# TUMFTM/DPFT

Hardware: AMD Instinct MI355X
Metric: training samples/sec (K-Radar C+R, bs4/GPU) (higher is better)
Workload: dtype f32

## Files before the change

### dpft_amd/csrc/decoder_train_x.hip

```cpp
#include "common.h"
#include "decoder_pack.h"
#include <stdlib.h>

namespace dpft {

constexpr int XR_DLIN = 0;
constexpr int XR_DF = XR_DLIN + NOA;
constexpr int XR_DPRE = XR_DF + 16;
constexpr int XR_DOUT = XR_DPRE + 32;
constexpr int XR_G3 = XR_DOUT + 16;
constexpr int XR_B3 = XR_G3 + 16;
constexpr int XR_G2 = XR_B3 + 16;
constexpr int XR_B2 = XR_G2 + 16;
constexpr int XR_DBV = XR_B2 + 16;
constexpr int XR_DVEC = XR_DBV + 16;
constexpr int XR_SUMMED = XR_DVEC + 16;
constexpr int XR_QP = XR_SUMMED;
constexpr int XR_HD = XR_QP + 16;
constexpr int XR_Y2 = XR_HD + 32;
constexpr int XR_VEC = XR_Y2 + 16;
constexpr int XR_SAMP = XR_VEC + 16;
constexpr int XR_FLOATS = XR_SAMP + 128;

struct Pyr5g {
    const float* level[DPFT_MAX_LEVELS];
    float* grad[DPFT_MAX_LEVELS];
    int H[DPFT_MAX_LEVELS], W[DPFT_MAX_LEVELS];
    int rep[DPFT_MAX_LEVELS];
    int L;
};
struct XfArgs {
    Pyr5g pyr[4];
    const float* pv[4];
    dpft_decoder_view raw[4];
    const float* y1;
    const float* pos;
    const float* ref;
    const int64_t* seed;
    float* y3;
    const float* dy3;
    float* dy1;
    float* dqp;
    float* dref;
    float* rows;
    float* fsave;
    float* scratch;
    signed char slot[4][DPFT_MAX_LEVELS];
    int B, Q, salt;
    int P[4];
    float p_drop;
    int exp;
};
constexpr int XS_ACC = 0;
constexpr int XS_MS = 128;
constexpr int XS_FLOATS = 136;
constexpr int XC_DS = 0;
constexpr int XC_SLOT = 128;
constexpr int XC_SLOT_FLOATS = 160;
constexpr int XC_MAX_SLOTS = 5;
constexpr int XC_FLOATS = XC_SLOT + XC_MAX_SLOTS * XC_SLOT_FLOATS;
constexpr int XC_MAX_PIXELS = 2048;

__device__ __forceinline__ uint32_t xdrop_hash(uint32_t idx, uint32_t s0, uint32_t s1) {
    uint32_t x = idx ^ s0;
    x *= 0xcc9e2d51u; x = (x << 15) | (x >> 17); x *= 0x1b873593u;
    x ^= s1;
    x ^= x >> 16; x *= 0x85ebca6bu; x ^= x >> 13; x *= 0xc2b2ae35u; x ^= x >> 16;
    return x;
}
__device__ __forceinline__ float xdrop_scale(const int64_t* seed, int salt, int stream_id, float p, uint32_t e) {
    const uint64_t s = (uint64_t)(*seed);
    const uint32_t s0 = (uint32_t)s ^ ((uint32_t)salt * 0x9E3779B9u);
    const uint32_t s1 = (uint32_t)(s >> 32) + (uint32_t)stream_id * 0x7F4A7C15u;
    const uint32_t thr = (uint32_t)(p * 65536.f + 0.5f);
    const uint32_t h = xdrop_hash(e >> 1, s0, s1);
    return ((h >> (16 * (e & 1))) & 0xFFFFu) >= thr ? 1.f / (1.f - p) : 0.f;
}

template <int CTRL>
__device__ __forceinline__ float xdpp(float v) {
    return __builtin_bit_cast(float, __builtin_amdgcn_update_dpp(0, __builtin_bit_cast(int, v), CTRL, 0xF, 0xF, false));
}
__device__ __forceinline__ float xg8_sum(float v) {
    v += xdpp<0xB1>(v);
    v += xdpp<0x4E>(v);
    v += xdpp<0x141>(v);
    return v;
}
__device__ __forceinline__ float xg16_sum(float v) {
    v = xg8_sum(v);
    v += xdpp<0x140>(v);
    return v;
}

struct XfFwd {
    float y1c;
    float mx, inv_den;
    float rx, ry;
    f32x2 acc;
    float ms;
    float vecc;
    float k2, y2, zhat2, rstd2;
    float pre, k3, hd;
    float k4, zhat3, rstd3, y3;
};

template <bool SAVED>
__device__ __forceinline__ void xf_forward_row(const XfArgs& a, int view, int bq, int b, int q, int lane, float* qp,
                                               float* lin, float* vec, XfFwd& f) {
    const float* pv = a.pv[view];
    const Pyr5g& pyr = a.pyr[view];
    const int L = pyr.L, P = a.P[view], LP = L * P;
    const size_t vbq = (size_t)view * a.B * a.Q + bq;
    const int c = lane & 15;
    f.y1c = a.y1[vbq * DC + c];
    if (lane < 16) qp[lane] = f.y1c + a.pos[(size_t)q * DC + lane];
    __builtin_amdgcn_wave_barrier();
    const int n_off = DM * LP * 2, n_all = DM * LP * 3;
    {
        float x[DC];
#pragma unroll
        for (int k = 0; k < DC; ++k) x[k] = qp[k];
        for (int o = lane; o < n_all; o += 64) {
            float s = pv[PV_OA_B + o];
#pragma unroll
            for (int k = 0; k < DC; ++k) s = fmaf(pv[PV_OA_WT + k * NOA + o], x[k], s);
            lin[o] = s;
        }
    }
    __builtin_amdgcn_wave_barrier();
    const int m = lane >> 3, j = lane & 7;
    const float* lg = lin + n_off + m * LP;
    float mx = -INFINITY;
    for (int i = 0; i < LP; ++i) mx = fmaxf(mx, lg[i]);
    float den = 0.f;
    for (int i = 0; i < LP; ++i) den += __expf(lg[i] - mx);
    f.mx = mx;
    f.inv_den = 1.f / den;
    f.rx = a.ref[vbq * 2 + 0];
    f.ry = a.ref[vbq * 2 + 1];
    const float* offp = lin + m * LP * 2;
    f32x2 acc = {0.f, 0.f};
    float ms = 0.f;
    if (SAVED) {
        const float* sv = a.fsave + vbq * XS_FLOATS;
        acc = *reinterpret_cast<const f32x2*>(sv + XS_ACC + m * DC + j * 2);
        ms = sv[XS_MS + m];
    }
    for (int l = 0; !SAVED && l < L; ++l) {
        const int H = pyr.H[l], W = pyr.W[l];
        const float* base = pyr.level[l] + (int64_t)b * H * W * DC + j * 2;
        f32x2 v[4][4];
        float wgt[4][4];
#pragma unroll
        for (int p = 0; p < 4; ++p) {
            const bool act = p < P;
            const int lp = act ? l * P + p : l * P;
            const float ox = offp[lp * 2 + 0], oy = offp[lp * 2 + 1];
            const float aw = act ? __expf(lg[lp] - mx) * f.inv_den : 0.f;
            const float lx = f.rx + ox / (float)W, ly = f.ry + oy / (float)H;
            const float h_im = ly * H - 0.5f, w_im = lx * W - 0.5f;
            const bool in = act && h_im > -1 && w_im > -1 && h_im < H && w_im < W;
            const float hf = floorf(h_im), wf = floorf(w_im);
            const int h_lo = (int)hf, w_lo = (int)wf, h_hi = h_lo + 1, w_hi = w_lo + 1;
            const float lh = h_im - hf, lw = w_im - wf, hh = 1 - lh, hw = 1 - lw;
            const bool k1 = in && h_lo >= 0 && w_lo >= 0, k2 = in && h_lo >= 0 && w_hi <= W - 1;
            const bool k3 = in && h_hi <= H - 1 && w_lo >= 0, k4 = in && h_hi <= H - 1 && w_hi <= W - 1;
            const int hl = min(max(h_lo, 0), H - 1), hh_ = min(max(h_hi, 0), H - 1);
            const int wl = min(max(w_lo, 0), W - 1), wh_ = min(max(w_hi, 0), W - 1);
            v[p][0] = *reinterpret_cast<const f32x2*>(base + ((int64_t)hl * W + wl) * DC);
            v[p][1] = *reinterpret_cast<const f32x2*>(base + ((int64_t)hl * W + wh_) * DC);
            v[p][2] = *reinterpret_cast<const f32x2*>(base + ((int64_t)hh_ * W + wl) * DC);
            v[p][3] = *reinterpret_cast<const f32x2*>(base + ((int64_t)hh_ * W + wh_) * DC);
            wgt[p][0] = k1 ? aw * hh * hw : 0.f;
            wgt[p][1] = k2 ? aw * hh * lw : 0.f;
            wgt[p][2] = k3 ? aw * lh * hw : 0.f;
            wgt[p][3] = k4 ? aw * lh * lw : 0.f;
        }
#pragma unroll
        for (int p = 0; p < 4; ++p)
#pragma unroll
            for (int k = 0; k < 4; ++k) {
                acc += wgt[p][k] * v[p][k];
                ms += wgt[p][k];
            }
    }
    f.acc = acc;
    f.ms = ms;
    const f32x2 wv0 = *reinterpret_cast<const f32x2*>(pv + PV_VAL_W + (m * DD + 0) * DC + j * 2);
    const f32x2 wv1 = *reinterpret_cast<const f32x2*>(pv + PV_VAL_W + (m * DD + 1) * DC + j * 2);
    const float o0 = xg8_sum(wv0[0] * acc[0] + wv0[1] * acc[1]);
    const float o1 = xg8_sum(wv1[0] * acc[0] + wv1[1] * acc[1]);
    if (j == 0) {
        vec[m * 2 + 0] = o0 + pv[PV_VAL_B + m * 2 + 0] * ms;
        vec[m * 2 + 1] = o1 + pv[PV_VAL_B + m * 2 + 1] * ms;
    }
    __builtin_amdgcn_wave_barrier();
    f.vecc = vec[c];
    float vo = pv[PV_OUTP_B + c];
#pragma unroll
    for (int k = 0; k < DC; ++k) vo = fmaf(pv[PV_OUTP_WT + k * DC + c], vec[k], vo);
    f.k2 = xdrop_scale(a.seed, a.salt, 2, a.p_drop, (uint32_t)(vbq * DC + c));
    vo = f.y1c + vo * f.k2;
    {
        const float mean = xg16_sum(vo) * (1.f / 16.f);
        const float d = vo - mean;
        const float var = xg16_sum(d * d) * (1.f / 16.f);
        f.rstd2 = 1.0f / sqrtf(var + 1e-5f);
        f.zhat2 = d * f.rstd2;
        f.y2 = f.zhat2 * pv[PV_N2_W + c] + pv[PV_N2_B + c];
    }
    __builtin_amdgcn_wave_barrier();
    if (lane < 16) qp[lane] = f.y2;
    __builtin_amdgcn_wave_barrier();
    {
        const int jf = lane & 31;
        float hsum = pv[PV_F1_B + jf];
#pragma unroll
        for (int k = 0; k < DC; ++k) hsum = fmaf(pv[PV_F1_WT + k * DFF + jf], qp[k], hsum);
        f.pre = hsum;
        f.k3 = xdrop_scale(a.seed, a.salt, 3, a.p_drop, (uint32_t)(vbq * DFF + jf));
        f.hd = mishf(hsum) * f.k3;
        if (lane < DFF) vec[lane] = f.hd;
    }
    __builtin_amdgcn_wave_barrier();
    float ff = pv[PV_F2_B + c];
#pragma unroll
    for (int k = 0; k < DFF; ++k) ff = fmaf(pv[PV_F2_WT + k * DC + c], vec[k], ff);
    f.k4 = xdrop_scale(a.seed, a.salt, 4, a.p_drop, (uint32_t)(vbq * DC + c));
    ff = f.y2 + ff * f.k4;
    {
        const float mean = xg16_sum(ff) * (1.f / 16.f);
        const float d = ff - mean;
        const float var = xg16_sum(d * d) * (1.f / 16.f);
        f.rstd3 = 1.0f / sqrtf(var + 1e-5f);
        f.zhat3 = d * f.rstd3;
        f.y3 = f.zhat3 * pv[PV_N3_W + c] + pv[PV_N3_B + c];
    }
}

constexpr int XF_WAVES = 5;
__global__ __launch_bounds__(256) void xf_train_fwd_kernel(XfArgs a) {
    __shared__ float sm[4][16 + NOA + 32];
    const int lane = threadIdx.x & 63, wv = __builtin_amdgcn_readfirstlane(threadIdx.x >> 6);
    const int bq = blockIdx.x * 4 + wv, view = blockIdx.y;
    if (bq >= a.B * a.Q) return;
    const int b = bq / a.Q, q = bq - b * a.Q;
    float* qp = sm[wv];
    XfFwd f;
    xf_forward_row<false>(a, view, bq, b, q, lane, qp, qp + 16, qp + 16 + NOA, f);
    const size_t vbq = (size_t)view * a.B * a.Q + bq;
    if (lane < 16) a.y3[vbq * DC + lane] = f.y3;
    if (a.fsave) {
        float* sv = a.fsave + vbq * XS_FLOATS;
        *reinterpret_cast<f32x2*>(sv + XS_ACC + (lane >> 3) * DC + (lane & 7) * 2) = f.acc;
        if ((lane & 7) == 0) sv[XS_MS + (lane >> 3)] = f.ms;
    }
}

template <bool SAVED>
__global__ __launch_bounds__(256, XF_WAVES) void xf_train_bwd_kernel(XfArgs a) {
    __shared__ __attribute__((aligned(16))) float sm[4][16 + NOA + 32 + NOA + 32 + 32 + 128 + 128 + 32];
    const int lane = threadIdx.x & 63, wv = __builtin_amdgcn_readfirstlane(threadIdx.x >> 6);
    const int bq = blockIdx.x * 4 + wv, view = blockIdx.y;
    if (bq >= a.B * a.Q) return;
    const int b = bq / a.Q, q = bq - b * a.Q;
    float* qp = sm[wv];
    float* lin = qp + 16;
    float* vec = lin + NOA;
    float* dlin = vec + 32;
    float* va = dlin + NOA;
    float* vb2 = va + 32;
    float* ds16 = vb2 + 32;
    float* sc_w = ds16 + 128;
    int* sc_o = reinterpret_cast<int*>(sc_w + 128);
    XfFwd f;
    xf_forward_row<SAVED>(a, view, bq, b, q, lane, qp, lin, vec, f);
    const float* pv = a.pv[view];
    const dpft_decoder_view& rw = a.raw[view];
    const Pyr5g& pyr = a.pyr[view];
    const int L = pyr.L, P = a.P[view], LP = L * P;
    const int n_off = DM * LP * 2, n_all = DM * LP * 3;
    const size_t vbq = (size_t)view * a.B * a.Q + bq;
    float* row = a.rows + vbq * XR_FLOATS;
    const int c = lane & 15, m = lane >> 3, j = lane & 7, jf = lane & 31;
    const bool w16 = lane < 16, w32 = lane < 32;
    const float dy3 = a.dy3[vbq * DC + c];
    float dzh = dy3 * pv[PV_N3_W + c];
    float m1 = xg16_sum(dzh) * (1.f / 16.f), m2 = xg16_sum(dzh * f.zhat3) * (1.f / 16.f);
    const float dz3 = f.rstd3 * (dzh - m1 - f.zhat3 * m2);
    const float df = dz3 * f.k4;
    if (w16) {
        row[XR_G3 + c] = dy3 * f.zhat3;
        row[XR_B3 + c] = dy3;
        row[XR_DF + c] = df;
        row[XR_Y2 + c] = f.y2;
        va[c] = df;
    }
    if (w32) row[XR_HD + jf] = f.hd;
    __builtin_amdgcn_wave_barrier();
    float dhd = 0.f;
#pragma unroll 4
    for (int k = 0; k < DC; ++k) dhd = fmaf(va[k], rw.ffn2_w[k * DFF + jf], dhd);
    float dpre;
    {
        const float x = f.pre;
        const float sp = x > 20.f ? x : log1pf(expf(x));
        const float t = tanhf(sp);
        const float sg = 1.f / (1.f + expf(-x));
        dpre = dhd * f.k3 * (t + x * (1.f - t * t) * sg);
    }
    if (w32) {
        row[XR_DPRE + jf] = dpre;
        vb2[jf] = dpre;
    }
    __builtin_amdgcn_wave_barrier();
    float dy2 = dz3;
#pragma unroll 4
    for (int k = 0; k < DFF; ++k) dy2 = fmaf(vb2[k], rw.ffn1_w[k * DC + c], dy2);
    dzh = dy2 * pv[PV_N2_W + c];
    m1 = xg16_sum(dzh) * (1.f / 16.f);
    m2 = xg16_sum(dzh * f.zhat2) * (1.f / 16.f);
    const float dz2 = f.rstd2 * (dzh - m1 - f.zhat2 * m2);
    const float dout = dz2 * f.k2;
    __builtin_amdgcn_wave_barrier();
    if (w16) {
        row[XR_G2 + c] = dy2 * f.zhat2;
        row[XR_B2 + c] = dy2;
        row[XR_DOUT + c] = dout;
        row[XR_VEC + c] = f.vecc;
        va[c] = dout;
    }
    __builtin_amdgcn_wave_barrier();
    float dvec = 0.f;
#pragma unroll 4
    for (int k = 0; k < DC; ++k) dvec = fmaf(va[k], rw.outp_w[k * DC + c], dvec);
    {
        const float msk = __shfl(f.ms, (c >> 1) * 8);
        if (w16) {
            row[XR_DVEC + c] = dvec;
            row[XR_DBV + c] = dvec * msk;
            vb2[c] = dvec;
        }
    }
    *reinterpret_cast<f32x2*>(row + XR_SAMP + m * DC + j * 2) = f.acc;
    __builtin_amdgcn_wave_barrier();
    const float g0 = vb2[m * DD + 0], g1 = vb2[m * DD + 1];
    const f32x2 w0 = *reinterpret_cast<const f32x2*>(pv + PV_VAL_W + (m * DD + 0) * DC + j * 2);
    const f32x2 w1v = *reinterpret_cast<const f32x2*>(pv + PV_VAL_W + (m * DD + 1) * DC + j * 2);
    const f32x2 dS = {w0[0] * g0 + w1v[0] * g1, w0[1] * g0 + w1v[1] * g1};
    const float dM = pv[PV_VAL_B + m * DD + 0] * g0 + pv[PV_VAL_B + m * DD + 1] * g1;
    *reinterpret_cast<f32x2*>(ds16 + m * DC + j * 2) = dS;
    float* rec = a.scratch ? a.scratch + vbq * XC_FLOATS : nullptr;
    if (rec) *reinterpret_cast<f32x2*>(rec + XC_DS + m * DC + j * 2) = dS;
    const float* lg = lin + n_off + m * LP;
    const float* offp = lin + m * LP * 2;
    float* dlg = dlin + n_off + m * LP;
    float* doff = dlin + m * LP * 2;
    float grx = 0.f, gry = 0.f, sdot = 0.f;
    for (int l = 0; l < L; ++l) {
        const int H = pyr.H[l], W = pyr.W[l];
        const float* base = pyr.level[l] + (int64_t)b * H * W * DC + j * 2;
        f32x2 v[4][4];
        float aw[4], hh[4], hw[4], lh[4], lw[4];
        bool kk[4][4];
#pragma unroll
        for (int p = 0; p < 4; ++p) {
            const bool act = p < P;
            const int lp = act ? l * P + p : l * P;
            const float ox = offp[lp * 2 + 0], oy = offp[lp * 2 + 1];
            aw[p] = act ? __expf(lg[lp] - f.mx) * f.inv_den : 0.f;
            const float lx = f.rx + ox / (float)W, ly = f.ry + oy / (float)H;
            const float h_im = ly * H - 0.5f, w_im = lx * W - 0.5f;
            const bool in = act && h_im > -1 && w_im > -1 && h_im < H && w_im < W;
            const float hf = floorf(h_im), wf = floorf(w_im);
            const int h_lo = (int)hf, w_lo = (int)wf, h_hi = h_lo + 1, w_hi = w_lo + 1;
            lh[p] = h_im - hf; lw[p] = w_im - wf; hh[p] = 1 - lh[p]; hw[p] = 1 - lw[p];
            kk[p][0] = in && h_lo >= 0 && w_lo >= 0;     kk[p][1] = in && h_lo >= 0 && w_hi <= W - 1;
            kk[p][2] = in && h_hi <= H - 1 && w_lo >= 0; kk[p][3] = in && h_hi <= H - 1 && w_hi <= W - 1;
            const int hl = min(max(h_lo, 0), H - 1), hh_ = min(max(h_hi, 0), H - 1);
            const int wl = min(max(w_lo, 0), W - 1), wh_ = min(max(w_hi, 0), W - 1);
            v[p][0] = *reinterpret_cast<const f32x2*>(base + ((int64_t)hl * W + wl) * DC);
            v[p][1] = *reinterpret_cast<const f32x2*>(base + ((int64_t)hl * W + wh_) * DC);
            v[p][2] = *reinterpret_cast<const f32x2*>(base + ((int64_t)hh_ * W + wl) * DC);
            v[p][3] = *reinterpret_cast<const f32x2*>(base + ((int64_t)hh_ * W + wh_) * DC);
            if (j == 0) {
                const float w1 = hh[p] * hw[p], w2 = hh[p] * lw[p], w3 = lh[p] * hw[p], w4 = lh[p] * lw[p];
                *reinterpret_cast<f32x4*>(sc_w + (p * 8 + m) * 4) =
                    f32x4{kk[p][0] ? aw[p] * w1 : 0.f, kk[p][1] ? aw[p] * w2 : 0.f, kk[p][2] ? aw[p] * w3 : 0.f,
                          kk[p][3] ? aw[p] * w4 : 0.f};
                sc_o[p * 8 + m] = in ? (h_lo * W + w_lo) * DC : 0;
            }
        }
#pragma unroll
        for (int p = 0; p < 4; ++p) {
            if (p >= P) break;
            const int lp = l * P + p;
            const float w1 = hh[p] * hw[p], w2 = hh[p] * lw[p], w3 = lh[p] * hw[p], w4 = lh[p] * lw[p];
            float ga = 0.f, gw = 0.f, gh = 0.f;
#pragma unroll
            for (int e = 0; e < 2; ++e) {
                const float v1 = kk[p][0] ? v[p][0][e] : 0.f, v2 = kk[p][1] ? v[p][1][e] : 0.f;
                const float v3 = kk[p][2] ? v[p][2][e] : 0.f, v4 = kk[p][3] ? v[p][3][e] : 0.f;
                ga += dS[e] * (w1 * v1 + w2 * v2 + w3 * v3 + w4 * v4);
                gh += dS[e] * aw[p] * (-hw[p] * v1 - lw[p] * v2 + hw[p] * v3 + lw[p] * v4);
                gw += dS[e] * aw[p] * (-hh[p] * v1 + hh[p] * v2 - lh[p] * v3 + lh[p] * v4);
            }
            if (j == 0) {
                const float i1 = kk[p][0] ? 1.f : 0.f, i2 = kk[p][1] ? 1.f : 0.f, i3 = kk[p][2] ? 1.f : 0.f, i4 = kk[p][3] ? 1.f : 0.f;
                ga += dM * (w1 * i1 + w2 * i2 + w3 * i3 + w4 * i4);
                gh += dM * aw[p] * (-hw[p] * i1 - lw[p] * i2 + hw[p] * i3 + lw[p] * i4);
                gw += dM * aw[p] * (-hh[p] * i1 + hh[p] * i2 - lh[p] * i3 + lh[p] * i4);
            }
            ga = xg8_sum(ga);
            gw = xg8_sum(gw);
            gh = xg8_sum(gh);
            sdot = fmaf(aw[p], ga, sdot);
            if (j == 0) {
                dlg[lp] = ga;
                doff[lp * 2 + 0] = gw;
                doff[lp * 2 + 1] = gh;
                grx = fmaf((float)W, gw, grx);
                gry = fmaf((float)H, gh, gry);
            }
        }
        __builtin_amdgcn_wave_barrier();
        const int slot = rec ? (int)a.slot[view][l] : -1;
        if (slot >= 0) {
            float* dst = rec + XC_SLOT + slot * XC_SLOT_FLOATS;
            if (lane < 32) reinterpret_cast<f32x4*>(dst)[lane] = reinterpret_cast<const f32x4*>(sc_w)[lane];
            else reinterpret_cast<int*>(dst + 128)[lane - 32] = sc_o[lane - 32];
        } else if (!(a.exp & 1)) {
            float* gl = pyr.grad[l] + (int64_t)(bq % pyr.rep[l]) * a.B * H * W * DC + (int64_t)b * H * W * DC;
            const int h4 = lane >> 4, ch = lane & 15, W16 = W * DC;
#pragma unroll
            for (int half = 0; half < 2; ++half) {
                const int m2 = h4 + 4 * half;
                const float val = ds16[m2 * DC + ch];
#pragma unroll
                for (int p = 0; p < 4; ++p) {
                    const f32x4 cw = *reinterpret_cast<const f32x4*>(sc_w + (p * 8 + m2) * 4);
                    float* g00 = gl + sc_o[p * 8 + m2] + ch;
                    if (cw[0] != 0.f) atomicAdd(g00, cw[0] * val);
                    if (cw[1] != 0.f) atomicAdd(g00 + DC, cw[1] * val);
                    if (cw[2] != 0.f) atomicAdd(g00 + W16, cw[2] * val);
                    if (cw[3] != 0.f) atomicAdd(g00 + W16 + DC, cw[3] * val);
                }
            }
        }
        __builtin_amdgcn_wave_barrier();
    }
    __builtin_amdgcn_wave_barrier();
    for (int lp = j; lp < LP; lp += 8) {
        const float awp = __expf(lg[lp] - f.mx) * f.inv_den;
        dlg[lp] = awp * (dlg[lp] - sdot);
    }
    {
        float sx = grx, sy = gry;
#pragma unroll
        for (int o = 8; o < 64; o <<= 1) {
            sx += __shfl_xor(sx, o);
            sy += __shfl_xor(sy, o);
        }
        if (lane == 0) {
            a.dref[vbq * 2 + 0] = sx;
            a.dref[vbq * 2 + 1] = sy;
        }
    }
    __builtin_amdgcn_wave_barrier();
    for (int o = lane; o < NOA; o += 64) row[XR_DLIN + o] = o < n_all ? dlin[o] : 0.f;
    const float qpc = f.y1c + a.pos[(size_t)q * DC + c];
    if (w16) row[XR_QP + c] = qpc;
    float dq = 0.f;
    {
        const int part = lane >> 4;
        for (int o = part; o < n_all; o += 4) {
            const float wgt = o < n_off ? rw.off_w[o * DC + c] : rw.att_w[(o - n_off) * DC + c];
            dq = fmaf(dlin[o], wgt, dq);
        }
        dq += __shfl_xor(dq, 16);
        dq += __shfl_xor(dq, 32);
    }
    if (w16) {
        a.dqp[vbq * DC + c] = dq;
        a.dy1[vbq * DC + c] = dz2 + dq;
    }
}

struct XsArgs {
    const float* scratch;
    float* grad[4 * XC_MAX_SLOTS];
    int H[4 * XC_MAX_SLOTS], W[4 * XC_MAX_SLOTS], view[4 * XC_MAX_SLOTS], slot[4 * XC_MAX_SLOTS];
    int B, Q, qchunk;
    int exp;
};
__global__ __launch_bounds__(512) void xf_scatter_small_kernel(XsArgs a) {
    extern __shared__ __attribute__((aligned(16))) float img[];
    const int tid = threadIdx.x, lane = tid & 63, wave = __builtin_amdgcn_readfirstlane(tid >> 6);
    const int mi = blockIdx.y, b = blockIdx.z;
    const int H = a.H[mi], W = a.W[mi], view = a.view[mi], slot = a.slot[mi];
    const int n = H * W * DC, W16 = W * DC;
    for (int i = tid * 4; i < n; i += 512 * 4) *reinterpret_cast<f32x4*>(img + i) = f32x4{0.f, 0.f, 0.f, 0.f};
    __syncthreads();
    const int q0 = blockIdx.x * a.qchunk, q1 = min(a.Q, q0 + a.qchunk);
    const int h4 = lane >> 4, ch = lane & 15;
    for (int q = q0 + wave; q < q1 && !(a.exp & 8); q += 8) {
        const float* rec = a.scratch + (((size_t)view * a.B + b) * a.Q + q) * XC_FLOATS;
        const float* wrec = rec + XC_SLOT + slot * XC_SLOT_FLOATS;
        const int* orec = reinterpret_cast<const int*>(wrec + 128);
        float val[2];
        f32x4 cw[2][4];
        int off[2][4];
#pragma unroll
        for (int half = 0; half < 2; ++half) {
            const int m2 = h4 + 4 * half;
            val[half] = rec[XC_DS + m2 * DC + ch];
#pragma unroll
            for (int p = 0; p < 4; ++p) {
                cw[half][p] = *reinterpret_cast<const f32x4*>(wrec + (p * 8 + m2) * 4);
                off[half][p] = orec[p * 8 + m2];
            }
        }
        if (a.exp & 2) {
            float acc = val[0] + val[1];
            for (int half = 0; half < 2; ++half)
                for (int p = 0; p < 4; ++p) acc += cw[half][p][0] + cw[half][p][3] + (float)off[half][p];
            if (acc == 12345.678f) img[0] = acc;
            continue;
        }
#pragma unroll
        for (int half = 0; half < 2; ++half)
#pragma unroll
            for (int p = 0; p < 4; ++p) {
                float* g00 = img + off[half][p] + ch;
                const f32x4 w4 = cw[half][p];
                if (w4[0] != 0.f) atomicAdd(g00, w4[0] * val[half]);
                if (w4[1] != 0.f) atomicAdd(g00 + DC, w4[1] * val[half]);
                if (w4[2] != 0.f) atomicAdd(g00 + W16, w4[2] * val[half]);
                if (w4[3] != 0.f) atomicAdd(g00 + W16 + DC, w4[3] * val[half]);
            }
    }
    __syncthreads();
    float* g = a.grad[mi] + (size_t)b * n;
    for (int i = tid; i < n && !(a.exp & 4); i += 512) {
        const float v = img[i];
        if (v != 0.f) atomicAdd(g + i, v);
    }
}

}

using namespace dpft;

static int xf_fill(XfArgs& a, const dpft_pyramid* pyr, const dpft_decoder_view* views, const float* packed, int V,
                   const int32_t* n_points, const float* y1, const float* pos, const float* ref, float p_drop,
                   const int64_t* seed, int salt, int B, int Q, bool need_grad) {
    DPFT_REQUIRE(pyr && views && packed && n_points && y1 && pos && ref && seed, "xattn_ffn_train: null argument");
    DPFT_REQUIRE(V >= 1 && V <= 4 && B > 0 && Q > 0, "xattn_ffn_train: bad sizes (V=%d, B=%d, Q=%d)", V, B, Q);
    DPFT_REQUIRE(p_drop >= 0.f && p_drop < 1.f, "xattn_ffn_train: dropout probability must be in [0,1)");
    DPFT_REQUIRE((int64_t)V * B * Q * DFF < (1ll << 32), "xattn_ffn_train: problem too large for the mask index");
    memset(&a, 0, sizeof(a));
    memset(a.slot, -1, sizeof(a.slot));
    for (int v = 0; v < V; ++v) {
        const dpft_pyramid* p = pyr + v;
        const int P = n_points[v];
        DPFT_REQUIRE(p->L >= 1 && p->L <= DPFT_MAX_LEVELS && P >= 1 && P <= 4 && p->L * P * DM * 3 <= NOA,
                     "xattn_ffn_train: L=%d, P=%d exceed the fused kernel's budget (P <= 4, L*P <= 20)", p->L, P);
        a.pyr[v].L = p->L;
        for (int l = 0; l < p->L; ++l) {
            DPFT_REQUIRE(p->level[l] && p->H[l] > 0 && p->W[l] > 0, "xattn_ffn_train: view %d level %d is invalid", v, l);
            DPFT_REQUIRE(!need_grad || p->grad[l], "xattn_ffn_train: view %d level %d has no gradient buffer", v, l);
            DPFT_REQUIRE((int64_t)p->H[l] * p->W[l] * DC < (1ll << 31), "xattn_ffn_train: view %d level %d is too large", v, l);
            a.pyr[v].level[l] = p->level[l]; a.pyr[v].grad[l] = p->grad[l];
            a.pyr[v].rep[l] = p->grad_replicas[l] > 1 ? p->grad_replicas[l] : 1;
            a.pyr[v].H[l] = p->H[l]; a.pyr[v].W[l] = p->W[l];
        }
        a.P[v] = P;
        a.pv[v] = packed + (size_t)v * PV_FLOATS;
        a.raw[v] = views[v];
    }
    a.y1 = y1; a.pos = pos; a.ref = ref; a.seed = seed; a.salt = salt; a.p_drop = p_drop; a.B = B; a.Q = Q;
    return DPFT_OK;
}

extern "C" int64_t dpft_xattn_ffn_train_row_floats(void) { return XR_FLOATS; }
extern "C" int64_t dpft_xattn_ffn_train_saved_floats(void) { return XS_FLOATS; }
extern "C" int64_t dpft_xattn_ffn_train_scratch_floats(void) { return XC_FLOATS; }

extern "C" int dpft_xattn_ffn_train_fwd_f32(const dpft_pyramid* pyr, const dpft_decoder_view* views, const float* packed,
                                            int32_t V, const int32_t* n_points, const float* y1, const float* pos,
                                            const float* ref, float p_drop, const int64_t* seed, int32_t salt, float* y3,
                                            float* saved, int32_t B, int32_t Q, dpft_stream_t stream) {
    XfArgs a;
    int rc = xf_fill(a, pyr, views, packed, V, n_points, y1, pos, ref, p_drop, seed, salt, B, Q, false);
    if (rc) return rc;
    DPFT_REQUIRE(y3, "xattn_ffn_train_fwd: null output");
    a.y3 = y3;
    a.fsave = saved;
    hipLaunchKernelGGL(xf_train_fwd_kernel, dim3(cdiv((int64_t)B * Q, 4), V), dim3(256), 0, (hipStream_t)stream, a);
    return check_launch("xattn_ffn_train_fwd");
}

extern "C" int dpft_xattn_ffn_train_bwd_f32(const dpft_pyramid* pyr, const dpft_decoder_view* views, const float* packed,
                                            int32_t V, const int32_t* n_points, const float* y1, const float* pos,
                                            const float* ref, float p_drop, const int64_t* seed, int32_t salt,
                                            const float* saved, const float* dy3, float* dy1, float* dqp, float* dref,
                                            float* rows, float* scratch, int32_t B, int32_t Q, dpft_stream_t stream) {
    XfArgs a;
    int rc = xf_fill(a, pyr, views, packed, V, n_points, y1, pos, ref, p_drop, seed, salt, B, Q, true);
    if (rc) return rc;
    DPFT_REQUIRE(dy3 && dy1 && dqp && dref && rows, "xattn_ffn_train_bwd: null argument");
    a.dy3 = dy3; a.dy1 = dy1; a.dqp = dqp; a.dref = dref; a.rows = rows;
    a.fsave = const_cast<float*>(saved);
    static const int exp = getenv("DPFT_XF_EXP") ? atoi(getenv("DPFT_XF_EXP")) : 0;
    a.exp = exp;
    XsArgs xs;
    memset(&xs, 0, sizeof(xs));
    int n_maps = 0, max_px = 0;
    static const bool allow = !(getenv("DPFT_XF_SCATTER") && atoi(getenv("DPFT_XF_SCATTER")) == 0);
    if (scratch && allow) {
        a.scratch = scratch;
        for (int v = 0; v < V; ++v) {
            int order[DPFT_MAX_LEVELS], n = 0;
            for (int l = 0; l < a.pyr[v].L; ++l)
                if (a.pyr[v].H[l] * a.pyr[v].W[l] <= XC_MAX_PIXELS && a.pyr[v].rep[l] == 1) order[n++] = l;
            for (int i = 1; i < n; ++i)
                for (int k = i; k > 0 && a.pyr[v].H[order[k]] * a.pyr[v].W[order[k]] < a.pyr[v].H[order[k - 1]] * a.pyr[v].W[order[k - 1]]; --k) {
                    const int t = order[k]; order[k] = order[k - 1]; order[k - 1] = t;
                }
            for (int i = 0; i < n && i < XC_MAX_SLOTS; ++i) {
                const int l = order[i];
                a.slot[v][l] = (signed char)i;
                xs.grad[n_maps] = a.pyr[v].grad[l];
                xs.H[n_maps] = a.pyr[v].H[l]; xs.W[n_maps] = a.pyr[v].W[l];
                xs.view[n_maps] = v; xs.slot[n_maps] = i;
                max_px = max_px > xs.H[n_maps] * xs.W[n_maps] ? max_px : xs.H[n_maps] * xs.W[n_maps];
                ++n_maps;
            }
        }
        if (n_maps == 0) a.scratch = nullptr;
    }
    if (saved)
        hipLaunchKernelGGL(xf_train_bwd_kernel<true>, dim3(cdiv((int64_t)B * Q, 4), V), dim3(256), 0, (hipStream_t)stream, a);
    else
        hipLaunchKernelGGL(xf_train_bwd_kernel<false>, dim3(cdiv((int64_t)B * Q, 4), V), dim3(256), 0, (hipStream_t)stream, a);
    rc = check_launch("xattn_ffn_train_bwd");
    if (rc || n_maps == 0) return rc;
    int nchunk = kNumCU / (n_maps * B);
    nchunk = nchunk < 1 ? 1 : (nchunk > 8 ? 8 : nchunk);
    xs.scratch = scratch; xs.B = B; xs.Q = Q; xs.qchunk = cdiv(Q, nchunk); xs.exp = exp;
    nchunk = cdiv(Q, xs.qchunk);
    const size_t lds = (size_t)max_px * DC * sizeof(float);
    static LdsGrant grant;
    (void)lds_grant(grant, reinterpret_cast<const void*>(xf_scatter_small_kernel), (size_t)XC_MAX_PIXELS * DC * sizeof(float));
    hipLaunchKernelGGL(xf_scatter_small_kernel, dim3(nchunk, n_maps, B), dim3(512), lds, (hipStream_t)stream, xs);
    return check_launch("xattn_ffn_train_bwd (small-map scatter)");
}
```

Baseline: 171.0.

## Stage decoder weights in LDS, vectorize GEMVs, and prefetch scatter records

Each block of the cross-attention forward and backward kernels now stages the value, out-projection, FFN and norm parameters into padded shared memory, and every per-row GEMV reads from there instead of global memory. The offset/attention linear layer is vectorized to float4 with register pinning. The dq reduction is split into chunked dot products, and the scatter path uses LDS address-space pointers plus an int-word read of the slot table. The small-scatter kernel software-pipelines record loads by prefetching the next query. These changes aim to cut global-memory and latency costs, at the price of a block-wide sync, extra LDS use and more register pressure.

Measured after the change: 167.0. 2.4% lower.

```diff
diff --git a/dpft_amd/csrc/decoder_train_x.hip b/dpft_amd/csrc/decoder_train_x.hip
--- a/dpft_amd/csrc/decoder_train_x.hip
+++ b/dpft_amd/csrc/decoder_train_x.hip
@@ -1,5 +1,6 @@
 #include "common.h"
 #include "decoder_pack.h"
+#include <stddef.h>
 #include <stdlib.h>
 
 namespace dpft {
@@ -68,8 +69,7 @@
     x ^= x >> 16; x *= 0x85ebca6bu; x ^= x >> 13; x *= 0xc2b2ae35u; x ^= x >> 16;
     return x;
 }
-__device__ __forceinline__ float xdrop_scale(const int64_t* seed, int salt, int stream_id, float p, uint32_t e) {
-    const uint64_t s = (uint64_t)(*seed);
+__device__ __forceinline__ float xdrop_scale(uint64_t s, int salt, int stream_id, float p, uint32_t e) {
     const uint32_t s0 = (uint32_t)s ^ ((uint32_t)salt * 0x9E3779B9u);
     const uint32_t s1 = (uint32_t)(s >> 32) + (uint32_t)stream_id * 0x7F4A7C15u;
     const uint32_t thr = (uint32_t)(p * 65536.f + 0.5f);
@@ -105,31 +105,107 @@
     float k4, zhat3, rstd3, y3;
 };
 
+constexpr int SW_VAL = 0;
+constexpr int SW_OUTP = SW_VAL + 272;
+constexpr int SW_F1 = SW_OUTP + 16 * 17;
+constexpr int SW_F2 = SW_F1 + 16 * 33;
+constexpr int SW_OUTP_B = SW_F2 + 32 * 17;
+constexpr int SW_N2_W = SW_OUTP_B + 16;
+constexpr int SW_N2_B = SW_N2_W + 16;
+constexpr int SW_F1_B = SW_N2_B + 16;
+constexpr int SW_F2_B = SW_F1_B + 32;
+constexpr int SW_N3_W = SW_F2_B + 16;
+constexpr int SW_N3_B = SW_N3_W + 16;
+constexpr int SW_FLOATS = SW_N3_B + 16;
+static_assert(PV_VAL_B == PV_VAL_W + 256 && PV_OUTP_WT == PV_VAL_W + 272 && PV_OUTP_B == PV_OUTP_WT + 256 &&
+              PV_F1_WT == PV_OUTP_B + 48 && PV_F1_B == PV_F1_WT + 512 && PV_F2_WT == PV_F1_B + 32 &&
+              PV_F2_B == PV_F2_WT + 512 && PV_FLOATS == PV_F2_B + 48 && PV_VAL_W % 4 == 0 && PV_FLOATS % 4 == 0 &&
+              PV_OA_WT % 4 == 0 && NOA % 4 == 0, "xf_stage_params / the float4 GEMV follow the packed layout");
+
+__device__ __forceinline__ int xf_stage_index(int r) {
+    constexpr int R_OUTP = PV_OUTP_WT - PV_VAL_W, R_OUTP_B = PV_OUTP_B - PV_VAL_W, R_F1 = PV_F1_WT - PV_VAL_W;
+    constexpr int R_F1_B = PV_F1_B - PV_VAL_W, R_F2 = PV_F2_WT - PV_VAL_W, R_F2_B = PV_F2_B - PV_VAL_W;
+    if (r < R_OUTP) return SW_VAL + r;
+    if (r < R_OUTP_B) return SW_OUTP + ((r - R_OUTP) >> 4) * 17 + ((r - R_OUTP) & 15);
+    if (r < R_F1) return SW_OUTP_B + (r - R_OUTP_B);
+    if (r < R_F1_B) return SW_F1 + ((r - R_F1) >> 5) * 33 + ((r - R_F1) & 31);
+    if (r < R_F2) return SW_F1_B + (r - R_F1_B);
+    if (r < R_F2_B) return SW_F2 + ((r - R_F2) >> 4) * 17 + ((r - R_F2) & 15);
+    return SW_F2_B + (r - R_F2_B);
+}
+__device__ __forceinline__ void xf_stage_params(const float* pv, float* sw) {
+    constexpr int N4 = (PV_FLOATS - PV_VAL_W) / 4;
+    const f32x4* src = reinterpret_cast<const f32x4*>(pv + PV_VAL_W);
+    const int t = threadIdx.x;
+    const f32x4 v0 = src[t];
+    const f32x4 v1 = src[t + 256 < N4 ? t + 256 : t];
+    const int d0 = xf_stage_index(t * 4);
+#pragma unroll
+    for (int e = 0; e < 4; ++e) sw[d0 + e] = v0[e];
+    if (t + 256 < N4) {
+        const int d1 = xf_stage_index((t + 256) * 4);
+#pragma unroll
+        for (int e = 0; e < 4; ++e) sw[d1 + e] = v1[e];
+    }
+    __syncthreads();
+}
+static_assert((PV_FLOATS - PV_VAL_W) / 4 > 256 && (PV_FLOATS - PV_VAL_W) / 4 <= 512, "xf_stage_params: two loads per thread");
+
+__device__ __forceinline__ void xf_pin8(f32x4 (&w)[8]) {
+    asm volatile("" : "+v"(w[0]), "+v"(w[1]), "+v"(w[2]), "+v"(w[3]), "+v"(w[4]), "+v"(w[5]), "+v"(w[6]), "+v"(w[7]));
+}
+typedef __attribute__((address_space(3))) const float xf_lds_f;
+typedef __attribute__((address_space(3))) const int xf_lds_i;
+template <class T>
+__device__ __forceinline__ T* xf_lds_pin(const void* p) {
+    T* q = (T*)p;
+    asm volatile("" : "+v"(q));
+    return q;
+}
+
 template <bool SAVED>
 __device__ __forceinline__ void xf_forward_row(const XfArgs& a, int view, int bq, int b, int q, int lane, float* qp,
-                                               float* lin, float* vec, XfFwd& f) {
+                                               float* lin, float* vec, const float* sw, XfFwd& f) {
     const float* pv = a.pv[view];
     const Pyr5g& pyr = a.pyr[view];
     const int L = pyr.L, P = a.P[view], LP = L * P;
     const size_t vbq = (size_t)view * a.B * a.Q + bq;
     const int c = lane & 15;
+    const int m = lane >> 3, j = lane & 7;
     f.y1c = a.y1[vbq * DC + c];
-    if (lane < 16) qp[lane] = f.y1c + a.pos[(size_t)q * DC + lane];
+    const float posc = a.pos[(size_t)q * DC + c];
+    f.rx = a.ref[vbq * 2 + 0];
+    f.ry = a.ref[vbq * 2 + 1];
+    const uint64_t seed = (uint64_t)(*a.seed);
+    f32x2 acc = {0.f, 0.f};
+    float ms = 0.f;
+    if (SAVED) {
+        const float* sv = a.fsave + vbq * XS_FLOATS;
+        acc = *reinterpret_cast<const f32x2*>(sv + XS_ACC + m * DC + j * 2);
+        ms = sv[XS_MS + m];
+    }
+    if (lane < 16) qp[lane] = f.y1c + posc;
     __builtin_amdgcn_wave_barrier();
     const int n_off = DM * LP * 2, n_all = DM * LP * 3;
-    {
-        float x[DC];
-#pragma unroll
-        for (int k = 0; k < DC; ++k) x[k] = qp[k];
-        for (int o = lane; o < n_all; o += 64) {
-            float s = pv[PV_OA_B + o];
-#pragma unroll
-            for (int k = 0; k < DC; ++k) s = fmaf(pv[PV_OA_WT + k * NOA + o], x[k], s);
-            lin[o] = s;
-        }
-    }
-    __builtin_amdgcn_wave_barrier();
-    const int m = lane >> 3, j = lane & 7;
+    for (int o = lane * 4; o < n_all; o += 256) {
+        const float* wt = pv + PV_OA_WT + o;
+        f32x4 s = *reinterpret_cast<const f32x4*>(pv + PV_OA_B + o);
+#pragma unroll
+        for (int k0 = 0; k0 < DC; k0 += 8) {
+            f32x4 w[8];
+#pragma unroll
+            for (int k = 0; k < 8; ++k) w[k] = *reinterpret_cast<const f32x4*>(wt + (k0 + k) * NOA);
+            xf_pin8(w);
+#pragma unroll
+            for (int k = 0; k < 8; ++k) {
+                const float x = qp[k0 + k];
+#pragma unroll
+                for (int e = 0; e < 4; ++e) s[e] = fmaf(w[k][e], x, s[e]);
+            }
+        }
+        *reinterpret_cast<f32x4*>(lin + o) = s;
+    }
+    __builtin_amdgcn_wave_barrier();
     const float* lg = lin + n_off + m * LP;
     float mx = -INFINITY;
     for (int i = 0; i < LP; ++i) mx = fmaxf(mx, lg[i]);
@@ -137,16 +213,7 @@
     for (int i = 0; i < LP; ++i) den += __expf(lg[i] - mx);
     f.mx = mx;
     f.inv_den = 1.f / den;
-    f.rx = a.ref[vbq * 2 + 0];
-    f.ry = a.ref[vbq * 2 + 1];
     const float* offp = lin + m * LP * 2;
-    f32x2 acc = {0.f, 0.f};
-    float ms = 0.f;
-    if (SAVED) {
-        const float* sv = a.fsave + vbq * XS_FLOATS;
-        acc = *reinterpret_cast<const f32x2*>(sv + XS_ACC + m * DC + j * 2);
-        ms = sv[XS_MS + m];
-    }
     for (int l = 0; !SAVED && l < L; ++l) {
         const int H = pyr.H[l], W = pyr.W[l];
         const float* base = pyr.level[l] + (int64_t)b * H * W * DC + j * 2;
@@ -187,20 +254,20 @@
     }
     f.acc = acc;
     f.ms = ms;
-    const f32x2 wv0 = *reinterpret_cast<const f32x2*>(pv + PV_VAL_W + (m * DD + 0) * DC + j * 2);
-    const f32x2 wv1 = *reinterpret_cast<const f32x2*>(pv + PV_VAL_W + (m * DD + 1) * DC + j * 2);
+    const f32x2 wv0 = *reinterpret_cast<const f32x2*>(sw + SW_VAL + (m * DD + 0) * DC + j * 2);
+    const f32x2 wv1 = *reinterpret_cast<const f32x2*>(sw + SW_VAL + (m * DD + 1) * DC + j * 2);
     const float o0 = xg8_sum(wv0[0] * acc[0] + wv0[1] * acc[1]);
     const float o1 = xg8_sum(wv1[0] * acc[0] + wv1[1] * acc[1]);
     if (j == 0) {
-        vec[m * 2 + 0] = o0 + pv[PV_VAL_B + m * 2 + 0] * ms;
-        vec[m * 2 + 1] = o1 + pv[PV_VAL_B + m * 2 + 1] * ms;
+        vec[m * 2 + 0] = o0 + sw[SW_VAL + 256 + m * 2 + 0] * ms;
+        vec[m * 2 + 1] = o1 + sw[SW_VAL + 256 + m * 2 + 1] * ms;
     }
     __builtin_amdgcn_wave_barrier();
     f.vecc = vec[c];
-    float vo = pv[PV_OUTP_B + c];
-#pragma unroll
-    for (int k = 0; k < DC; ++k) vo = fmaf(pv[PV_OUTP_WT + k * DC + c], vec[k], vo);
-    f.k2 = xdrop_scale(a.seed, a.salt, 2, a.p_drop, (uint32_t)(vbq * DC + c));
+    float vo = sw[SW_OUTP_B + c];
+#pragma unroll
+    for (int k = 0; k < DC; ++k) vo = fmaf(sw[SW_OUTP + k * 17 + c], vec[k], vo);
+    f.k2 = xdrop_scale(seed, a.salt, 2, a.p_drop, (uint32_t)(vbq * DC + c));
     vo = f.y1c + vo * f.k2;
     {
         const float mean = xg16_sum(vo) * (1.f / 16.f);
@@ -208,26 +275,26 @@
         const float var = xg16_sum(d * d) * (1.f / 16.f);
         f.rstd2 = 1.0f / sqrtf(var + 1e-5f);
         f.zhat2 = d * f.rstd2;
-        f.y2 = f.zhat2 * pv[PV_N2_W + c] + pv[PV_N2_B + c];
+        f.y2 = f.zhat2 * sw[SW_N2_W + c] + sw[SW_N2_B + c];
     }
     __builtin_amdgcn_wave_barrier();
     if (lane < 16) qp[lane] = f.y2;
     __builtin_amdgcn_wave_barrier();
     {
         const int jf = lane & 31;
-        float hsum = pv[PV_F1_B + jf];
-#pragma unroll
-        for (int k = 0; k < DC; ++k) hsum = fmaf(pv[PV_F1_WT + k * DFF + jf], qp[k], hsum);
+        float hsum = sw[SW_F1_B + jf];
+#pragma unroll
+        for (int k = 0; k < DC; ++k) hsum = fmaf(sw[SW_F1 + k * 33 + jf], qp[k], hsum);
         f.pre = hsum;
-        f.k3 = xdrop_scale(a.seed, a.salt, 3, a.p_drop, (uint32_t)(vbq * DFF + jf));
+        f.k3 = xdrop_scale(seed, a.salt, 3, a.p_drop, (uint32_t)(vbq * DFF + jf));
         f.hd = mishf(hsum) * f.k3;
         if (lane < DFF) vec[lane] = f.hd;
     }
     __builtin_amdgcn_wave_barrier();
-    float ff = pv[PV_F2_B + c];
-#pragma unroll
-    for (int k = 0; k < DFF; ++k) ff = fmaf(pv[PV_F2_WT + k * DC + c], vec[k], ff);
-    f.k4 = xdrop_scale(a.seed, a.salt, 4, a.p_drop, (uint32_t)(vbq * DC + c));
+    float ff = sw[SW_F2_B + c];
+#pragma unroll
+    for (int k = 0; k < DFF; ++k) ff = fmaf(sw[SW_F2 + k * 17 + c], vec[k], ff);
+    f.k4 = xdrop_scale(seed, a.salt, 4, a.p_drop, (uint32_t)(vbq * DC + c));
     ff = f.y2 + ff * f.k4;
     {
         const float mean = xg16_sum(ff) * (1.f / 16.f);
@@ -235,20 +302,22 @@
         const float var = xg16_sum(d * d) * (1.f / 16.f);
         f.rstd3 = 1.0f / sqrtf(var + 1e-5f);
         f.zhat3 = d * f.rstd3;
-        f.y3 = f.zhat3 * pv[PV_N3_W + c] + pv[PV_N3_B + c];
+        f.y3 = f.zhat3 * sw[SW_N3_W + c] + sw[SW_N3_B + c];
     }
 }
 
 constexpr int XF_WAVES = 5;
 __global__ __launch_bounds__(256) void xf_train_fwd_kernel(XfArgs a) {
-    __shared__ float sm[4][16 + NOA + 32];
+    __shared__ __attribute__((aligned(16))) float sm[4][16 + NOA + 32];
+    __shared__ float sw[SW_FLOATS];
     const int lane = threadIdx.x & 63, wv = __builtin_amdgcn_readfirstlane(threadIdx.x >> 6);
     const int bq = blockIdx.x * 4 + wv, view = blockIdx.y;
+    xf_stage_params(a.pv[view], sw);
     if (bq >= a.B * a.Q) return;
     const int b = bq / a.Q, q = bq - b * a.Q;
     float* qp = sm[wv];
     XfFwd f;
-    xf_forward_row<false>(a, view, bq, b, q, lane, qp, qp + 16, qp + 16 + NOA, f);
+    xf_forward_row<false>(a, view, bq, b, q, lane, qp, qp + 16, qp + 16 + NOA, sw, f);
     const size_t vbq = (size_t)view * a.B * a.Q + bq;
     if (lane < 16) a.y3[vbq * DC + lane] = f.y3;
     if (a.fsave) {
@@ -258,11 +327,30 @@
     }
 }
 
+template <int CH>
+__device__ __forceinline__ float xf_dot_chunk(const float* w, const float* d, float dq) {
+    float t[CH];
+#pragma unroll
+    for (int u = 0; u < CH; ++u) t[u] = w[u * 4 * DC];
+#pragma unroll
+    for (int u = 0; u < CH; ++u) dq = fmaf(d[u * 4], t[u], dq);
+    return dq;
+}
+__device__ __forceinline__ float xf_dot_rows(const float* w, const float* d, int n, float dq) {
+    int i = 0;
+    for (; i + 16 <= n; i += 16) dq = xf_dot_chunk<16>(w + i * 4 * DC, d + i * 4, dq);
+    for (; i + 4 <= n; i += 4) dq = xf_dot_chunk<4>(w + i * 4 * DC, d + i * 4, dq);
+    for (; i < n; i += 2) dq = xf_dot_chunk<2>(w + i * 4 * DC, d + i * 4, dq);
+    return dq;
+}
+
 template <bool SAVED>
 __global__ __launch_bounds__(256, XF_WAVES) void xf_train_bwd_kernel(XfArgs a) {
     __shared__ __attribute__((aligned(16))) float sm[4][16 + NOA + 32 + NOA + 32 + 32 + 128 + 128 + 32];
+    __shared__ float sw[SW_FLOATS];
     const int lane = threadIdx.x & 63, wv = __builtin_amdgcn_readfirstlane(threadIdx.x >> 6);
     const int bq = blockIdx.x * 4 + wv, view = blockIdx.y;
+    xf_stage_params(a.pv[view], sw);
     if (bq >= a.B * a.Q) return;
     const int b = bq / a.Q, q = bq - b * a.Q;
     float* qp = sm[wv];
@@ -275,8 +363,7 @@
     float* sc_w = ds16 + 128;
     int* sc_o = reinterpret_cast<int*>(sc_w + 128);
     XfFwd f;
-    xf_forward_row<SAVED>(a, view, bq, b, q, lane, qp, lin, vec, f);
-    const float* pv = a.pv[view];
+    xf_forward_row<SAVED>(a, view, bq, b, q, lane, qp, lin, vec, sw, f);
     const dpft_decoder_view& rw = a.raw[view];
     const Pyr5g& pyr = a.pyr[view];
     const int L = pyr.L, P = a.P[view], LP = L * P;
@@ -286,7 +373,7 @@
     const int c = lane & 15, m = lane >> 3, j = lane & 7, jf = lane & 31;
     const bool w16 = lane < 16, w32 = lane < 32;
     const float dy3 = a.dy3[vbq * DC + c];
-    float dzh = dy3 * pv[PV_N3_W + c];
+    float dzh = dy3 * sw[SW_N3_W + c];
     float m1 = xg16_sum(dzh) * (1.f / 16.f), m2 = xg16_sum(dzh * f.zhat3) * (1.f / 16.f);
     const float dz3 = f.rstd3 * (dzh - m1 - f.zhat3 * m2);
     const float df = dz3 * f.k4;
@@ -300,8 +387,8 @@
     if (w32) row[XR_HD + jf] = f.hd;
     __builtin_amdgcn_wave_barrier();
     float dhd = 0.f;
-#pragma unroll 4
-    for (int k = 0; k < DC; ++k) dhd = fmaf(va[k], rw.ffn2_w[k * DFF + jf], dhd);
+#pragma unroll
+    for (int k = 0; k < DC; ++k) dhd = fmaf(va[k], sw[SW_F2 + jf * 17 + k], dhd);
     float dpre;
     {
         const float x = f.pre;
@@ -316,9 +403,9 @@
     }
     __builtin_amdgcn_wave_barrier();
     float dy2 = dz3;
-#pragma unroll 4
-    for (int k = 0; k < DFF; ++k) dy2 = fmaf(vb2[k], rw.ffn1_w[k * DC + c], dy2);
-    dzh = dy2 * pv[PV_N2_W + c];
+#pragma unroll
+    for (int k = 0; k < DFF; ++k) dy2 = fmaf(vb2[k], sw[SW_F1 + c * 33 + k], dy2);
+    dzh = dy2 * sw[SW_N2_W + c];
     m1 = xg16_sum(dzh) * (1.f / 16.f);
     m2 = xg16_sum(dzh * f.zhat2) * (1.f / 16.f);
     const float dz2 = f.rstd2 * (dzh - m1 - f.zhat2 * m2);
@@ -330,11 +417,13 @@
         row[XR_DOUT + c] = dout;
         row[XR_VEC + c] = f.vecc;
         va[c] = dout;
+        vec[c] = dz2;
+        vec[DC + c] = f.y1c;
     }
     __builtin_amdgcn_wave_barrier();
     float dvec = 0.f;
-#pragma unroll 4
-    for (int k = 0; k < DC; ++k) dvec = fmaf(va[k], rw.outp_w[k * DC + c], dvec);
+#pragma unroll
+    for (int k = 0; k < DC; ++k) dvec = fmaf(va[k], sw[SW_OUTP + c * 17 + k], dvec);
     {
         const float msk = __shfl(f.ms, (c >> 1) * 8);
         if (w16) {
@@ -346,10 +435,10 @@
     *reinterpret_cast<f32x2*>(row + XR_SAMP + m * DC + j * 2) = f.acc;
     __builtin_amdgcn_wave_barrier();
     const float g0 = vb2[m * DD + 0], g1 = vb2[m * DD + 1];
-    const f32x2 w0 = *reinterpret_cast<const f32x2*>(pv + PV_VAL_W + (m * DD + 0) * DC + j * 2);
-    const f32x2 w1v = *reinterpret_cast<const f32x2*>(pv + PV_VAL_W + (m * DD + 1) * DC + j * 2);
+    const f32x2 w0 = *reinterpret_cast<const f32x2*>(sw + SW_VAL + (m * DD + 0) * DC + j * 2);
+    const f32x2 w1v = *reinterpret_cast<const f32x2*>(sw + SW_VAL + (m * DD + 1) * DC + j * 2);
     const f32x2 dS = {w0[0] * g0 + w1v[0] * g1, w0[1] * g0 + w1v[1] * g1};
-    const float dM = pv[PV_VAL_B + m * DD + 0] * g0 + pv[PV_VAL_B + m * DD + 1] * g1;
+    const float dM = sw[SW_VAL + 256 + m * DD + 0] * g0 + sw[SW_VAL + 256 + m * DD + 1] * g1;
     *reinterpret_cast<f32x2*>(ds16 + m * DC + j * 2) = dS;
     float* rec = a.scratch ? a.scratch + vbq * XC_FLOATS : nullptr;
     if (rec) *reinterpret_cast<f32x2*>(rec + XC_DS + m * DC + j * 2) = dS;
@@ -360,7 +449,7 @@
     float grx = 0.f, gry = 0.f, sdot = 0.f;
     for (int l = 0; l < L; ++l) {
         const int H = pyr.H[l], W = pyr.W[l];
-        const float* base = pyr.level[l] + (int64_t)b * H * W * DC + j * 2;
+        const float* base = pyr.level[l] + (int64_t)b * H * W * DC;
         f32x2 v[4][4];
         float aw[4], hh[4], hw[4], lh[4], lw[4];
         bool kk[4][4];
@@ -380,10 +469,10 @@
             kk[p][2] = in && h_hi <= H - 1 && w_lo >= 0; kk[p][3] = in && h_hi <= H - 1 && w_hi <= W - 1;
             const int hl = min(max(h_lo, 0), H - 1), hh_ = min(max(h_hi, 0), H - 1);
             const int wl = min(max(w_lo, 0), W - 1), wh_ = min(max(w_hi, 0), W - 1);
-            v[p][0] = *reinterpret_cast<const f32x2*>(base + ((int64_t)hl * W + wl) * DC);
-            v[p][1] = *reinterpret_cast<const f32x2*>(base + ((int64_t)hl * W + wh_) * DC);
-            v[p][2] = *reinterpret_cast<const f32x2*>(base + ((int64_t)hh_ * W + wl) * DC);
-            v[p][3] = *reinterpret_cast<const f32x2*>(base + ((int64_t)hh_ * W + wh_) * DC);
+            v[p][0] = *reinterpret_cast<const f32x2*>(base + ((hl * W + wl) * DC + j * 2));
+            v[p][1] = *reinterpret_cast<const f32x2*>(base + ((hl * W + wh_) * DC + j * 2));
+            v[p][2] = *reinterpret_cast<const f32x2*>(base + ((hh_ * W + wl) * DC + j * 2));
+            v[p][3] = *reinterpret_cast<const f32x2*>(base + ((hh_ * W + wh_) * DC + j * 2));
             if (j == 0) {
                 const float w1 = hh[p] * hw[p], w2 = hh[p] * lw[p], w3 = lh[p] * hw[p], w4 = lh[p] * lw[p];
                 *reinterpret_cast<f32x4*>(sc_w + (p * 8 + m) * 4) =
@@ -425,22 +514,32 @@
             }
         }
         __builtin_amdgcn_wave_barrier();
-        const int slot = rec ? (int)a.slot[view][l] : -1;
+        int slot = -1;
+        if (rec) {
+            static_assert(sizeof(a.slot) % 4 == 0 && offsetof(XfArgs, slot) % 4 == 0, "slot is read by words");
+            const int si = view * DPFT_MAX_LEVELS + l;
+            const int word = reinterpret_cast<const int*>(&a.slot[0][0])[si >> 2];
+            slot = (int)(signed char)(word >> ((si & 3) * 8));
+        }
         if (slot >= 0) {
             float* dst = rec + XC_SLOT + slot * XC_SLOT_FLOATS;
             if (lane < 32) reinterpret_cast<f32x4*>(dst)[lane] = reinterpret_cast<const f32x4*>(sc_w)[lane];
             else reinterpret_cast<int*>(dst + 128)[lane - 32] = sc_o[lane - 32];
         } else if (!(a.exp & 1)) {
             float* gl = pyr.grad[l] + (int64_t)(bq % pyr.rep[l]) * a.B * H * W * DC + (int64_t)b * H * W * DC;
-            const int h4 = lane >> 4, ch = lane & 15, W16 = W * DC;
+            int ln = lane;
+            asm volatile("" : "+v"(ln));
+            const int h4 = ln >> 4, ch = ln & 15, W16 = W * DC;
+            xf_lds_f* ds_l = xf_lds_pin<xf_lds_f>(ds16 + ln);
+            xf_lds_f* cw_l = xf_lds_pin<xf_lds_f>(sc_w + h4 * 4);
+            xf_lds_i* co_l = xf_lds_pin<xf_lds_i>(sc_o + h4);
 #pragma unroll
             for (int half = 0; half < 2; ++half) {
-                const int m2 = h4 + 4 * half;
-                const float val = ds16[m2 * DC + ch];
+                const float val = ds_l[half * 64];
 #pragma unroll
                 for (int p = 0; p < 4; ++p) {
-                    const f32x4 cw = *reinterpret_cast<const f32x4*>(sc_w + (p * 8 + m2) * 4);
-                    float* g00 = gl + sc_o[p * 8 + m2] + ch;
+                    const f32x4 cw = *reinterpret_cast<__attribute__((address_space(3))) const f32x4*>(cw_l + (p * 8 + 4 * half) * 4);
+                    float* g00 = gl + (co_l[p * 8 + 4 * half] + ch);
                     if (cw[0] != 0.f) atomicAdd(g00, cw[0] * val);
                     if (cw[1] != 0.f) atomicAdd(g00 + DC, cw[1] * val);
                     if (cw[2] != 0.f) atomicAdd(g00 + W16, cw[2] * val);
@@ -469,21 +568,19 @@
     }
     __builtin_amdgcn_wave_barrier();
     for (int o = lane; o < NOA; o += 64) row[XR_DLIN + o] = o < n_all ? dlin[o] : 0.f;
-    const float qpc = f.y1c + a.pos[(size_t)q * DC + c];
+    const float qpc = vec[DC + c] + a.pos[(size_t)q * DC + c];
     if (w16) row[XR_QP + c] = qpc;
     float dq = 0.f;
     {
         const int part = lane >> 4;
-        for (int o = part; o < n_all; o += 4) {
-            const float wgt = o < n_off ? rw.off_w[o * DC + c] : rw.att_w[(o - n_off) * DC + c];
-            dq = fmaf(dlin[o], wgt, dq);
-        }
+        dq = xf_dot_rows(rw.off_w + part * DC + c, dlin + part, n_off >> 2, dq);
+        dq = xf_dot_rows(rw.att_w + part * DC + c, dlin + n_off + part, (n_all - n_off) >> 2, dq);
         dq += __shfl_xor(dq, 16);
         dq += __shfl_xor(dq, 32);
     }
     if (w16) {
         a.dqp[vbq * DC + c] = dq;
-        a.dy1[vbq * DC + c] = dz2 + dq;
+        a.dy1[vbq * DC + c] = vec[c] + dq;
     }
 }
 
@@ -494,6 +591,25 @@
     int B, Q, qchunk;
     int exp;
 };
+struct XsRecord {
+    float val[2];
+    f32x4 cw[2][4];
+    int off[2][4];
+};
+__device__ __forceinline__ void xs_load_record(XsRecord& r, const float* rec, int slot, int h4, int ch) {
+    const float* wrec = rec + XC_SLOT + slot * XC_SLOT_FLOATS;
+    const int* orec = reinterpret_cast<const int*>(wrec + 128);
+#pragma unroll
+    for (int half = 0; half < 2; ++half) {
+        const int m2 = h4 + 4 * half;
+        r.val[half] = rec[XC_DS + m2 * DC + ch];
+#pragma unroll
+        for (int p = 0; p < 4; ++p) {
+            r.cw[half][p] = *reinterpret_cast<const f32x4*>(wrec + (p * 8 + m2) * 4);
+            r.off[half][p] = orec[p * 8 + m2];
+        }
+    }
+}
 __global__ __launch_bounds__(512) void xf_scatter_small_kernel(XsArgs a) {
     extern __shared__ __attribute__((aligned(16))) float img[];
     const int tid = threadIdx.x, lane = tid & 63, wave = __builtin_amdgcn_readfirstlane(tid >> 6);
@@ -504,27 +620,17 @@
     __syncthreads();
     const int q0 = blockIdx.x * a.qchunk, q1 = min(a.Q, q0 + a.qchunk);
     const int h4 = lane >> 4, ch = lane & 15;
-    for (int q = q0 + wave; q < q1 && !(a.exp & 8); q += 8) {
-        const float* rec = a.scratch + (((size_t)view * a.B + b) * a.Q + q) * XC_FLOATS;
-        const float* wrec = rec + XC_SLOT + slot * XC_SLOT_FLOATS;
-        const int* orec = reinterpret_cast<const int*>(wrec + 128);
-        float val[2];
-        f32x4 cw[2][4];
-        int off[2][4];
-#pragma unroll
-        for (int half = 0; half < 2; ++half) {
-            const int m2 = h4 + 4 * half;
-            val[half] = rec[XC_DS + m2 * DC + ch];
-#pragma unroll
-            for (int p = 0; p < 4; ++p) {
-                cw[half][p] = *reinterpret_cast<const f32x4*>(wrec + (p * 8 + m2) * 4);
-                off[half][p] = orec[p * 8 + m2];
-            }
-        }
+    XsRecord cur, nxt;
+    const size_t rec0 = ((size_t)view * a.B + b) * a.Q;
+    const bool rows_on = !(a.exp & 8);
+    if (rows_on && q0 + wave < q1) xs_load_record(nxt, a.scratch + (rec0 + q0 + wave) * XC_FLOATS, slot, h4, ch);
+    for (int q = q0 + wave; q < q1 && rows_on; q += 8) {
+        cur = nxt;
+        if (q + 8 < q1) xs_load_record(nxt, a.scratch + (rec0 + q + 8) * XC_FLOATS, slot, h4, ch);
         if (a.exp & 2) {
-            float acc = val[0] + val[1];
+            float acc = cur.val[0] + cur.val[1];
             for (int half = 0; half < 2; ++half)
-                for (int p = 0; p < 4; ++p) acc += cw[half][p][0] + cw[half][p][3] + (float)off[half][p];
+                for (int p = 0; p < 4; ++p) acc += cur.cw[half][p][0] + cur.cw[half][p][3] + (float)cur.off[half][p];
             if (acc == 12345.678f) img[0] = acc;
             continue;
         }
@@ -532,12 +638,12 @@
         for (int half = 0; half < 2; ++half)
 #pragma unroll
             for (int p = 0; p < 4; ++p) {
-                float* g00 = img + off[half][p] + ch;
-                const f32x4 w4 = cw[half][p];
-                if (w4[0] != 0.f) atomicAdd(g00, w4[0] * val[half]);
-                if (w4[1] != 0.f) atomicAdd(g00 + DC, w4[1] * val[half]);
-                if (w4[2] != 0.f) atomicAdd(g00 + W16, w4[2] * val[half]);
-                if (w4[3] != 0.f) atomicAdd(g00 + W16 + DC, w4[3] * val[half]);
+                float* g00 = img + cur.off[half][p] + ch;
+                const f32x4 w4 = cur.cw[half][p];
+                if (w4[0] != 0.f) atomicAdd(g00, w4[0] * cur.val[half]);
+                if (w4[1] != 0.f) atomicAdd(g00 + DC, w4[1] * cur.val[half]);
+                if (w4[2] != 0.f) atomicAdd(g00 + W16, w4[2] * cur.val[half]);
+                if (w4[3] != 0.f) atomicAdd(g00 + W16 + DC, w4[3] * cur.val[half]);
             }
     }
     __syncthreads();
```
